# in5omnia/Image_Segmentation

Hardware: AMD Instinct MI355X
Metric: images/sec (fwd+bwd) U-Net 3-class 256x256; IoU parity vs CPU ref (higher is better)
Workload: dtype bf16; 1 GPU; unet(3,3) train step (fwd + ce + bwd + grad all-reduce + AdamW), B=32/GPU 3x256x256, BASELINE config 2; global_batch=32, parallelism=dp1, rccl_ranks=0, rehearsal=False

## Files before the change

image_segmentation_amd/csrc/wgrad.hip:

```cpp
#include <stdlib.h>
#include <type_traits>
#include "common.hpp"
#include "segk_internal.h"
#include "../../include/segk.h"

namespace {

template <int I, int N, typename F> __device__ __forceinline__ void static_for(F&& f) {
  if constexpr (I < N) {
    f(std::integral_constant<int, I>{});
    static_for<I + 1, N>(f);
  }
}

template <typename T, int GEO, int WC = 1> struct WG {
  static constexpr bool BF = (sizeof(T) == 2);
  static constexpr int R = (GEO == 2) ? (BF ? (WC == 4 ? 8 : 4) : 2) : (BF ? 8 : 4);
  static constexpr int NTAPS = GEO == 0 ? 9 : (GEO == 1 ? 1 : 4);
  static constexpr int PH = GEO == 0 ? R + 2 : (GEO == 1 ? R : 2 * R);
  static constexpr int PW = GEO == 0 ? 18 : (GEO == 1 ? 16 : 32);
  static constexpr int BLKP = 32 * (int)sizeof(T);
  static constexpr int PPB = BLKP / 16;
  static constexpr int NDZ = R * 16;
  static constexpr int NPP = PH * PW;
};

__device__ __forceinline__ int tap_pixel(int geo, int tap, int r, int x) {
  if (geo == 0) return (r + tap / 3) * 18 + x + tap % 3;
  if (geo == 1) return r * 16 + x;
  return (2 * r + (tap >> 1)) * 32 + 2 * x + (tap & 1);
}

template <typename T, int GEO, int WC, int WI>
__global__ __launch_bounds__((WC * WI > 4 ? WC * WI : 4) * 64, (sizeof(T) == 2 ? 2 : 1)) void wgrad_kernel(const WgradArgs a) {
  using G = WG<T, GEO, WC>;
  using E = ET<T>;
  constexpr int NT = (WC * WI > 4 ? WC * WI : 4) * 64;
  constexpr int R = G::R, NTAPS = G::NTAPS, BLKP = G::BLKP, PPB = G::PPB;
  constexpr int DZ_PIECES = G::NDZ * WC * PPB, PA_PIECES = G::NPP * WI * PPB;
  constexpr int NDL = (DZ_PIECES + NT - 1) / NT, NPL = (PA_PIECES + NT - 1) / NT;
  constexpr int DZ_BYTES = WC * G::NDZ * BLKP;

  extern __shared__ __attribute__((aligned(16))) char smem[];
  char* const dzs = smem;
  char* const pas = smem + DZ_BYTES;

  const int tid = threadIdx.x, lane = tid & 63, wave = tid >> 6;
  const int H = a.H, W = a.W;
  const int tiles_x = (W + 15) >> 4, tiles_y = (H + R - 1) / R;
  const int ntiles = a.B * tiles_y * tiles_x;

  const int KT = (a.CA + a.CB) / (32 * WI), NCT = (a.CD / (32 * WC)) * KT;
  const int lid = xcd_remap(blockIdx.x, gridDim.x);
  const int s = lid / NCT, ct = lid - s * NCT;
  const int n0 = (ct / KT) * 32 * WC, k0 = (ct % KT) * 32 * WI;

  const T* src; int SC, kc0;
  if (k0 < a.CA) { src = (const T*)a.srcA; SC = a.CA; kc0 = k0; }
  else { src = (const T*)a.srcB; SC = a.CB; kc0 = k0 - a.CA; }
  const bool pro = (a.scale != nullptr);
  const int FH = GEO == 2 ? 2 * H : H, FW = GEO == 2 ? 2 * W : W;

  static_assert(NT % (WC * PPB) == 0 && NT % (WI * PPB) == 0, "channel slot must be thread-invariant");
  const int dcc = tid % (WC * PPB), pcc = tid % (WI * PPB);
  int d_pix[NDL], p_pix[NPL];
#pragma unroll
  for (int i = 0; i < NDL; ++i) {
    const int q = tid + i * NT;
    d_pix[i] = q < DZ_PIECES ? q / (WC * PPB) : -1;
  }
#pragma unroll
  for (int i = 0; i < NPL; ++i) {
    const int q = tid + i * NT;
    p_pix[i] = q < PA_PIECES ? q / (WI * PPB) : -1;
  }
  float psc[E::VEC], psh[E::VEC];
  if (pro) {
#pragma unroll
    for (int j = 0; j < E::VEC; ++j) {
      psc[j] = a.scale[kc0 + pcc * E::VEC + j];
      psh[j] = a.shift[kc0 + pcc * E::VEC + j];
    }
  }

  uint4 dreg[NDL], preg[NPL];
  bool pok[NPL];
  auto prefetch = [&](int t) {
    const int b = t / (tiles_y * tiles_x);
    const int rem = t - b * tiles_y * tiles_x;
    const int y0 = (rem / tiles_x) * R, x0 = (rem % tiles_x) * 16;
#pragma unroll
    for (int i = 0; i < NDL; ++i) {
      uint4 v = make_uint4(0, 0, 0, 0);
      if (d_pix[i] >= 0) {
        const int gy = y0 + (d_pix[i] >> 4), gx = x0 + (d_pix[i] & 15);
        if (gy < H && gx < W)
          v = *(const uint4*)((const T*)a.dz + ((size_t)(b * H + gy) * W + gx) * a.CD + n0 + dcc * E::VEC);
      }
      dreg[i] = v;
    }
#pragma unroll
    for (int i = 0; i < NPL; ++i) {
      pok[i] = false;
      uint4 v = make_uint4(0, 0, 0, 0);
      if (p_pix[i] >= 0) {
        const int py = p_pix[i] / G::PW, px = p_pix[i] - py * G::PW;
        int gy, gx;
        if (GEO == 0) { gy = y0 + py - 1; gx = x0 + px - 1; }
        else if (GEO == 1) { gy = y0 + py; gx = x0 + px; }
        else { gy = 2 * y0 + py; gx = 2 * x0 + px; }
        if (gy >= 0 && gy < FH && gx >= 0 && gx < FW) {
          pok[i] = true;
          v = *(const uint4*)(src + ((size_t)(b * FH + gy) * FW + gx) * SC + kc0 + pcc * E::VEC);
        }
      }
      preg[i] = v;
    }
  };
  auto stage = [&]() {
#pragma unroll
    for (int i = 0; i < NDL; ++i)
      if (d_pix[i] >= 0) {
        const int blk = dcc / PPB, c16 = dcc - blk * PPB;
        *(uint4*)(dzs + blk * (G::NDZ * BLKP) + d_pix[i] * BLKP + c16 * 16) = dreg[i];
      }
#pragma unroll
    for (int i = 0; i < NPL; ++i)
      if (p_pix[i] >= 0) {
        const int blk = pcc / PPB, c16 = pcc - blk * PPB;
        uint4 v = make_uint4(0, 0, 0, 0);
        if (pok[i]) {
          v = preg[i];
          if (pro) {
            float f[E::VEC];
            unpack16<T>(v, f);
#pragma unroll
            for (int j = 0; j < E::VEC; ++j) f[j] = fmaxf(fmaf(f[j], psc[j], psh[j]), 0.f);
            v = pack16<T>(f);
          }
        }
        *(uint4*)(pas + blk * (G::NPP * BLKP) + p_pix[i] * BLKP + c16 * 16) = v;
      }
  };

  const bool computes = wave < WC * WI;
  const int wc = wave / WI, wi = wave - wc * WI;
  f32x16 acc[NTAPS];
#pragma unroll
  for (int t = 0; t < NTAPS; ++t)
#pragma unroll
    for (int r = 0; r < 16; ++r) acc[t][r] = 0.f;

  const char* const dzb = dzs + wc * (G::NDZ * BLKP);
  const char* const pab = pas + wi * (G::NPP * BLKP);

  int t = s;
  if (t < ntiles) prefetch(t);
  for (; t < ntiles; t += a.S) {
    stage();
    __syncthreads();
    if (t + a.S < ntiles) prefetch(t + a.S);
    if (computes) {
      if constexpr (G::BF) {
        const int g = lane >> 4, i16 = lane & 15, q = i16 >> 2, p = i16 & 3;
        const int gsub = g & 1, h = g >> 1;
        const int coff = (16 * gsub + 4 * p) * 2;
        if constexpr (GEO == 2) {
          typedef __attribute__((address_space(3))) s16x4* lds_v4;
          const int xa = 8 * h + q;
          bf16x8 fa[R], fb[2][NTAPS];
          auto rd_b = [&](int r, bf16x8 (&F)[NTAPS]) {
#pragma unroll
            for (int tp = 0; tp < NTAPS; ++tp) {
              const int p0 = tap_pixel(GEO, tp, r, xa), p1 = tap_pixel(GEO, tp, r, xa + 4);
              const s16x4 b0 = __builtin_amdgcn_ds_read_tr16_b64_v4i16((lds_v4)(pab + p0 * BLKP + coff));
              const s16x4 b1 = __builtin_amdgcn_ds_read_tr16_b64_v4i16((lds_v4)(pab + p1 * BLKP + coff));
              F[tp] = __builtin_bit_cast(bf16x8, __builtin_shufflevector(b0, b1, 0, 1, 2, 3, 4, 5, 6, 7));
            }
          };
#pragma unroll
          for (int r = 0; r < R; ++r) {
            const s16x4 a0 = __builtin_amdgcn_ds_read_tr16_b64_v4i16((lds_v4)(dzb + (r * 16 + xa) * BLKP + coff));
            const s16x4 a1 = __builtin_amdgcn_ds_read_tr16_b64_v4i16((lds_v4)(dzb + (r * 16 + xa + 4) * BLKP + coff));
            fa[r] = __builtin_bit_cast(bf16x8, __builtin_shufflevector(a0, a1, 0, 1, 2, 3, 4, 5, 6, 7));
          }
          rd_b(0, fb[0]);
#pragma unroll
          for (int r = 0; r < R; ++r) {
            if (r + 1 < R) rd_b(r + 1, fb[(r + 1) & 1]);
            __builtin_amdgcn_sched_barrier(0);
#pragma unroll
            for (int tp = 0; tp < NTAPS; ++tp) acc[tp] = __builtin_amdgcn_mfma_f32_32x32x16_bf16(fa[r], fb[r & 1][tp], acc[tp], 0, 0, 0);
            __builtin_amdgcn_sched_barrier(0);
          }
        } else {
      #pragma unroll
        for (int r = 0; r < R; ++r) {
          const int xa = 8 * h + q;
          typedef __attribute__((address_space(3))) s16x4* lds_v4;
          const s16x4 a0 = __builtin_amdgcn_ds_read_tr16_b64_v4i16((lds_v4)(dzb + (r * 16 + xa) * BLKP + coff));
          const s16x4 a1 = __builtin_amdgcn_ds_read_tr16_b64_v4i16((lds_v4)(dzb + (r * 16 + xa + 4) * BLKP + coff));
          const bf16x8 fa = __builtin_bit_cast(bf16x8, __builtin_shufflevector(a0, a1, 0, 1, 2, 3, 4, 5, 6, 7));
#pragma unroll
          for (int tp = 0; tp < NTAPS; ++tp) {
            const int p0 = tap_pixel(GEO, tp, r, xa), p1 = tap_pixel(GEO, tp, r, xa + 4);
            const s16x4 b0 = __builtin_amdgcn_ds_read_tr16_b64_v4i16((lds_v4)(pab + p0 * BLKP + coff));
            const s16x4 b1 = __builtin_amdgcn_ds_read_tr16_b64_v4i16((lds_v4)(pab + p1 * BLKP + coff));
            const bf16x8 fb = __builtin_bit_cast(bf16x8, __builtin_shufflevector(b0, b1, 0, 1, 2, 3, 4, 5, 6, 7));
            acc[tp] = __builtin_amdgcn_mfma_f32_32x32x16_bf16(fa, fb, acc[tp], 0, 0, 0);
          }
        }
        }
      } else {
        const int i32 = lane & 31, h = lane >> 5;
#pragma unroll
        for (int r = 0; r < R; ++r) {
#pragma unroll
          for (int kp = 0; kp < 8; ++kp) {
            const int x = 2 * kp + h;
            const float fa = *(const float*)(dzb + (r * 16 + x) * BLKP + i32 * 4);
#pragma unroll
            for (int tp = 0; tp < NTAPS; ++tp) {
              const float fb = *(const float*)(pab + tap_pixel(GEO, tp, r, x) * BLKP + i32 * 4);
              acc[tp] = __builtin_amdgcn_mfma_f32_32x32x2f32(fa, fb, acc[tp], 0, 0, 0);
            }
          }
        }
      }
    }
    __syncthreads();
  }

  if (computes) {
    const int K = a.CA + a.CB;
    const int col = lane & 31, lh = lane >> 5;
    float* const slab = a.slabs + (size_t)s * a.CD * NTAPS * K;
#pragma unroll
    for (int tp = 0; tp < NTAPS; ++tp)
#pragma unroll
      for (int r = 0; r < 16; ++r) {
        const int row = (r & 3) + 8 * (r >> 2) + 4 * lh;
        slab[((size_t)(n0 + wc * 32 + row) * NTAPS + tp) * K + k0 + wi * 32 + col] = acc[tp][r];
      }
  }
}

#ifdef SEGK_WGRAD_STAMPS
__device__ unsigned long long g_wstamps[256 * 8 * 8];
#endif
template <int WC, int WI, bool PRO, bool RAG>
__global__ __launch_bounds__((WC * WI > 4 ? WC * WI : 4) * 64, 2) void wgrad_dma_kernel(const WgradArgs a) {
  typedef bf16_t T;
  constexpr int NWV = WC * WI > 4 ? WC * WI : 4;
  constexpr int R = 8, NTAPS = 9, BLKP = 64;
  constexpr int WU = PRO ? WI : WC, WV = PRO ? WC : WI;
  constexpr int NU = R * 16, NV = 192;
  constexpr int UB = WU * NU * BLKP, VB = WV * NV * BLKP, BUF = UB + VB;
  constexpr int NINSTR = WU * 8 + WV * 12;
  extern __shared__ __attribute__((aligned(16))) char smem[];

  const int tid = threadIdx.x, lane = tid & 63;
  const int wave = __builtin_amdgcn_readfirstlane(tid >> 6);
  const int H = a.H, W = a.W;
  const int tiles_x = (W + 15) >> 4, tiles_y = (H + R - 1) / R;
  const int ntiles = a.B * tiles_y * tiles_x;
  const int KT = (a.CA + a.CB) / (32 * WI), NCT = (a.CD / (32 * WC)) * KT;
  const int lid = xcd_remap(blockIdx.x, gridDim.x);
  const int s = lid / NCT, ct = lid - s * NCT;
  const int n0 = (ct / KT) * 32 * WC, k0 = (ct % KT) * 32 * WI;

  const T* srck; int SCk, kc0;
  if (k0 < a.CA) { srck = (const T*)a.srcA; SCk = a.CA; kc0 = k0; }
  else { srck = (const T*)a.srcB; SCk = a.CB; kc0 = k0 - a.CA; }
  const T* const ubase = PRO ? srck + kc0 : (const T*)a.dz + n0;
  const int UC = PRO ? SCk : a.CD;
  const T* const vbase = PRO ? (const T*)a.dz + n0 : srck + kc0;
  const int VC = PRO ? a.CD : SCk;
  const char* const zeros = (const char*)a.zeros;

  const int lp = lane >> 2, lc = lane & 3;
  constexpr int NI = (NINSTR + NWV - 1) / NWV;
  int poff[NI];
  int pyx[RAG ? NI : 1];
  unsigned pflag[(NI + 5) / 6];
#pragma unroll
  for (int q = 0; q < (NI + 5) / 6; ++q) pflag[q] = 0u;
#pragma unroll
  for (int i = 0; i < NI; ++i) {
    const int j = min(wave + NWV * i, NINSTR - 1);
    if (j < WU * 8) {
      const int blk = j >> 3, r = j & 7;
      poff[i] = ((r * W + lp) * UC + blk * 32 + lc * 8) * 2;
      if constexpr (RAG) pyx[i] = ((r + 1) << 8) | (lp + 1);
    } else {
      const int jj = j - WU * 8;
      const int blk = jj / 12, ch = jj - blk * 12;
      const int pp = ch * 16 + lp;
      const int py = pp / 18, px = pp - py * 18;
      poff[i] = (((py - 1) * W + (px - 1)) * VC + blk * 32 + lc * 8) * 2;
      const unsigned f = (py == 0 ? 1u : 0u) | (py == 9 ? 2u : 0u) | (px == 0 ? 4u : 0u) | (px == 17 ? 8u : 0u) |
                         (pp >= 180 ? 16u : 0u);
      pflag[i / 6] |= f << (5 * (i % 6));
      if constexpr (RAG) pyx[i] = (py << 8) | px;
    }
  }
  auto issue_tile = [&](int t, int bufsel) {
    const int bimg = t / (tiles_y * tiles_x);
    const int rem = t - bimg * tiles_y * tiles_x;
    const int y0 = (rem / tiles_x) * R, x0 = (rem % tiles_x) * 16;
    {
      const unsigned out = (y0 == 0 ? 1u : 0u) | (y0 + R >= H ? 2u : 0u) | (x0 == 0 ? 4u : 0u) | (x0 + 16 >= W ? 8u : 0u) | 16u;
      const size_t pix0 = (size_t)(bimg * H + y0) * W + x0;
      const char* const ub0 = (const char*)(ubase + pix0 * UC);
      const char* const vb0 = (const char*)(vbase + pix0 * VC);
      char* const bb = smem + bufsel * BUF;
      const char* const zsrc = zeros + lc * 16;
#pragma unroll
      for (int i = 0; i < NI; ++i) {
        const int j = wave + NWV * i;
        if (j >= NINSTR) break;
        const bool is_u = j < WU * 8;
        const int jj = j - WU * 8;
        char* const dst = is_u ? bb + (j >> 3) * (NU * BLKP) + (j & 7) * 1024
                               : bb + UB + (jj / 12) * (NV * BLKP) + (jj % 12) * 1024;
        const char* const base = is_u ? ub0 : vb0;
        bool bad;
        if constexpr (RAG) {
          const int py = pyx[i] >> 8, px = pyx[i] & 255;
          bad = (((pflag[i / 6] >> (5 * (i % 6))) & 16u) != 0u) | (py == 0 ? y0 == 0 : py > H - y0) |
                (px == 0 ? x0 == 0 : px > W - x0);
        } else {
          bad = ((pflag[i / 6] >> (5 * (i % 6))) & out) != 0u;
        }
        const char* const src = bad ? zsrc : base + (ptrdiff_t)poff[i];
        __builtin_amdgcn_global_load_lds((const __attribute__((address_space(1))) void*)src,
                                         (__attribute__((address_space(3))) void*)dst, 16, 0, 0);
      }
    }
  };

  const bool computes = wave < WC * WI;
  const int wc = wave / WI, wi = wave - wc * WI;
  const int wu = PRO ? wi : wc, wv = PRO ? wc : wi;
  f32x16 acc[NTAPS];
#pragma unroll
  for (int t = 0; t < NTAPS; ++t)
#pragma unroll
    for (int r = 0; r < 16; ++r) acc[t][r] = 0.f;

  const int g = lane >> 4, i16 = lane & 15, q = i16 >> 2, p = i16 & 3;
  const int gsub = g & 1, h = g >> 1;
  const int coff = (16 * gsub + 4 * p) * 2;
  const int xa = 8 * h + q;
  float psc = 1.f, psh = 0.f;
  if (PRO) {
    const int c = kc0 + wu * 32 + 16 * gsub + i16;
    psc = a.scale[c];
    psh = a.shift[c];
  }
  typedef __attribute__((ext_vector_type(8))) short s16x8;
  auto frag_rd = [&](s16x8& dst, int vaddr, auto OFFc) {
    constexpr int OFF = decltype(OFFc)::value;
    s16x4 f0, f1;
    asm volatile("ds_read_b64_tr_b16 %0, %1 offset:%2" : "=v"(f0) : "v"(vaddr), "n"(OFF));
    asm volatile("ds_read_b64_tr_b16 %0, %1 offset:%2" : "=v"(f1) : "v"(vaddr), "n"(OFF + 4 * BLKP));
    dst = __builtin_shufflevector(f0, f1, 0, 1, 2, 3, 4, 5, 6, 7);
  };
  typedef short s16x2 __attribute__((ext_vector_type(2)));
  auto transform = [&](s16x8 v, unsigned vmask) {
    const uint4 raw = __builtin_bit_cast(uint4, v);
    float f[8];
    unpack16<T>(raw, f);
    unsigned o[4];
#pragma unroll
    for (int i = 0; i < 4; ++i) {
      const float x0 = fmaf(f[2 * i], psc, psh), x1 = fmaf(f[2 * i + 1], psc, psh);
      unsigned pk;
      pk = cvt_pk_bf16(x0, x1);
      o[i] = __builtin_bit_cast(unsigned, __builtin_elementwise_max(__builtin_bit_cast(s16x2, pk), (s16x2){0, 0}));
    }
    if (vmask != 0xffu) {
#pragma unroll
      for (int i = 0; i < 4; ++i)
        o[i] &= ((vmask >> (2 * i)) & 1 ? 0x0000ffffu : 0u) | ((vmask >> (2 * i + 1)) & 1 ? 0xffff0000u : 0u);
    }
    return __builtin_bit_cast(s16x8, make_uint4(o[0], o[1], o[2], o[3]));
  };

#ifdef SEGK_WGRAD_STAMPS
  unsigned long long wst[3] = {0, 0, 0}, wlast, wt0;
  asm volatile("s_waitcnt lgkmcnt(0)\n\ts_memtime %0\n\ts_waitcnt lgkmcnt(0)" : "=s"(wlast)::"memory");
  wt0 = wlast;
#define WSTAMP(i) do { unsigned long long t_; asm volatile("s_memtime %0\n\ts_waitcnt lgkmcnt(0)" : "=s"(t_)::"memory"); \
                       wst[i] += t_ - wlast; wlast = t_; } while (0)
#else
#define WSTAMP(i) do {} while (0)
#endif
  int t = s, cur = 0;
  if (t < ntiles) issue_tile(t, 0);
  asm volatile("s_waitcnt vmcnt(0)" ::: "memory");
  __syncthreads();
  WSTAMP(2);
#ifndef WGRAD_STAGGER_ROW
#define WGRAD_STAGGER_ROW 1
#endif
  constexpr int SROW = (NWV == 8) ? WGRAD_STAGGER_ROW : -1;
  const bool late_issue = SROW >= 0 && wave >= NWV / 2;
  for (; t < ntiles; t += a.S) {
    const bool has_next = t + a.S < ntiles;
    if (has_next && !late_issue) issue_tile(t + a.S, cur ^ 1);
    if (computes) {
      unsigned xmask = 0xffu, rows_ok = R;
      if (PRO) {
        const int bimg = t / (tiles_y * tiles_x);
        const int rem = t - bimg * tiles_y * tiles_x;
        const int y0 = (rem / tiles_x) * R, x0 = (rem % tiles_x) * 16;
        rows_ok = (unsigned)min(R, H - y0);
        xmask = 0;
#pragma unroll
        for (int j = 0; j < 8; ++j)
          xmask |= (x0 + 8 * h + j < W ? 1u : 0u) << j;
      }
      const int ua = cur * BUF + wu * (NU * BLKP) + xa * BLKP + coff;
      const int va = cur * BUF + UB + wv * (NV * BLKP) + xa * BLKP + coff;
      s16x8 fv[3][3], fu[2];
      frag_rd(fu[0], ua, std::integral_constant<int, 0>{});
      static_for<0, 9>([&](auto IC) {
        constexpr int y = decltype(IC)::value / 3, kx = decltype(IC)::value % 3;
        frag_rd(fv[y][kx], va, std::integral_constant<int, (y * 18 + kx) * BLKP>{});
      });
      if (PRO) {
        asm volatile("s_waitcnt lgkmcnt(15)" ::: "memory");
        __builtin_amdgcn_sched_barrier(0);
        fu[0] = transform(fu[0], rows_ok > 0 ? xmask : 0u);
      }
      static_for<0, R>([&](auto RC) {
        constexpr int r = decltype(RC)::value;
        if constexpr (r + 1 < R) frag_rd(fu[(r + 1) & 1], ua, std::integral_constant<int, (r + 1) * 16 * BLKP>{});
        asm volatile("s_waitcnt lgkmcnt(%0)" ::"n"((r == 0 ? 12 : 6) + (r + 1 < R ? 2 : 0)) : "memory");
        __builtin_amdgcn_sched_barrier(0);
        const bf16x8 fur = __builtin_bit_cast(bf16x8, fu[r & 1]);
#pragma unroll
        for (int kx = 0; kx < 3; ++kx) {
          const bf16x8 fvr = __builtin_bit_cast(bf16x8, fv[r % 3][kx]);
          const int ti = PRO ? 8 - kx : kx;
          acc[ti] = PRO ? __builtin_amdgcn_mfma_f32_32x32x16_bf16(fvr, fur, acc[ti], 0, 0, 0)
                        : __builtin_amdgcn_mfma_f32_32x32x16_bf16(fur, fvr, acc[ti], 0, 0, 0);
        }
        __builtin_amdgcn_sched_barrier(0);
        if constexpr (r + 1 < R) {
          static_for<0, 3>([&](auto KC) {
            constexpr int kx = decltype(KC)::value;
            frag_rd(fv[r % 3][kx], va, std::integral_constant<int, ((r + 3) * 18 + kx) * BLKP>{});
          });
        }
        asm volatile("s_waitcnt lgkmcnt(%0)" ::"n"(r + 1 < R ? 8 : 0) : "memory");
        __builtin_amdgcn_sched_barrier(0);
#pragma unroll
        for (int ky = 1; ky < 3; ++ky)
#pragma unroll
          for (int kx = 0; kx < 3; ++kx) {
            const bf16x8 fvr = __builtin_bit_cast(bf16x8, fv[(r + ky) % 3][kx]);
            const int ti = PRO ? 8 - (ky * 3 + kx) : ky * 3 + kx;
            acc[ti] = PRO ? __builtin_amdgcn_mfma_f32_32x32x16_bf16(fvr, fur, acc[ti], 0, 0, 0)
                          : __builtin_amdgcn_mfma_f32_32x32x16_bf16(fur, fvr, acc[ti], 0, 0, 0);
          }
        __builtin_amdgcn_sched_barrier(0);
        if constexpr (r == SROW) {
          if (has_next && late_issue) issue_tile(t + a.S, cur ^ 1);
          __builtin_amdgcn_sched_barrier(0);
        }
        if constexpr (PRO && r + 1 < R) {
          asm volatile("s_waitcnt lgkmcnt(6)" ::: "memory");
          __builtin_amdgcn_sched_barrier(0);
          fu[(r + 1) & 1] = transform(fu[(r + 1) & 1], (unsigned)(r + 1) < rows_ok ? xmask : 0u);
        }
      });
    }
    WSTAMP(0);
    asm volatile("s_waitcnt vmcnt(0)" ::: "memory");
    WSTAMP(1);
    __syncthreads();
    WSTAMP(2);
    cur ^= 1;
  }

  if (computes) {
    const int K = a.CA + a.CB;
    const int col = lane & 31, lh = lane >> 5;
    float* const slab = a.slabs + (size_t)s * a.CD * NTAPS * K;
#pragma unroll
    for (int tp = 0; tp < NTAPS; ++tp)
#pragma unroll
      for (int r = 0; r < 16; ++r) {
        const int row = (r & 3) + 8 * (r >> 2) + 4 * lh;
        slab[((size_t)(n0 + wc * 32 + row) * NTAPS + tp) * K + k0 + wi * 32 + col] = acc[tp][r];
      }
  }
#ifdef SEGK_WGRAD_STAMPS
  {
    unsigned long long t_;
    asm volatile("s_waitcnt vmcnt(0)\n\ts_memtime %0\n\ts_waitcnt lgkmcnt(0)" : "=s"(t_)::"memory");
    if (lane == 0 && blockIdx.x < 256) {
      unsigned long long* o = g_wstamps + ((size_t)blockIdx.x * 8 + wave) * 8;
      o[0] = wst[0]; o[1] = wst[1]; o[2] = wst[2]; o[3] = t_ - wlast; o[4] = t_ - wt0;
    }
  }
#endif
}

template <int WC, int WI, bool PRO, bool RAG>
int launch_dma(const WgradArgs& a, hipStream_t st) {
  constexpr int WU = PRO ? WI : WC, WV = PRO ? WC : WI;
  constexpr size_t lds = 2 * ((size_t)WU * 128 * 64 + (size_t)WV * 192 * 64);
  static_assert(lds <= 160 * 1024, "wgrad_dma: LDS exceeds 160 KiB");
  const int NCT = (a.CD / (32 * WC)) * ((a.CA + a.CB) / (32 * WI));
  auto kern = wgrad_dma_kernel<WC, WI, PRO, RAG>;
  static bool attr_set[SEGK_MAX_DEVICES] = {};
  const int dev_ = segk_device_index();
  if (!attr_set[dev_]) {
    if (hipFuncSetAttribute((const void*)kern, hipFuncAttributeMaxDynamicSharedMemorySize, 160 * 1024) != hipSuccess)
      SEGK_FAIL(-3, "wgrad_dma: cannot raise dynamic LDS limit");
    attr_set[dev_] = true;
  }
  hipLaunchKernelGGL(kern, dim3(a.S * NCT), dim3((WC * WI > 4 ? WC * WI : 4) * 64), lds, st, a);
#ifdef SEGK_WGRAD_STAMPS
  { void* sp = nullptr; if (hipGetSymbolAddress(&sp, HIP_SYMBOL(g_wstamps)) == hipSuccess) (void)hipMemcpyAsync(a.slabs, sp, sizeof(unsigned long long) * 256 * 8 * 8, hipMemcpyDeviceToDevice, st); }
#endif
  SEGK_CHECK_LAUNCH("wgrad_dma");
  return 0;
}

template <int WC, int WI>
int launch_dma_pro(const WgradArgs& a, hipStream_t st) {
  const bool rag = a.H % 8 != 0 || a.W % 16 != 0;
  if (rag) return a.scale ? launch_dma<WC, WI, true, true>(a, st) : launch_dma<WC, WI, false, true>(a, st);
  return a.scale ? launch_dma<WC, WI, true, false>(a, st) : launch_dma<WC, WI, false, false>(a, st);
}

template <typename T, int GEO, int WC, int WI>
int launch_cfg(const WgradArgs& a, hipStream_t st) {
  using G = WG<T, GEO, WC>;
  const size_t lds = (size_t)WC * G::NDZ * G::BLKP + (size_t)WI * G::NPP * G::BLKP;
  const int NCT = (a.CD / (32 * WC)) * ((a.CA + a.CB) / (32 * WI));
  auto kern = wgrad_kernel<T, GEO, WC, WI>;
  static bool attr_set[SEGK_MAX_DEVICES] = {};
  const int dev_ = segk_device_index();
  if (!attr_set[dev_]) {
    if (hipFuncSetAttribute((const void*)kern, hipFuncAttributeMaxDynamicSharedMemorySize, 160 * 1024) != hipSuccess)
      SEGK_FAIL(-3, "wgrad: cannot raise dynamic LDS limit");
    attr_set[dev_] = true;
  }
  hipLaunchKernelGGL(kern, dim3(a.S * NCT), dim3((WC * WI > 4 ? WC * WI : 4) * 64), lds, st, a);
#ifdef SEGK_WGRAD_STAMPS
  { void* sp = nullptr; if (hipGetSymbolAddress(&sp, HIP_SYMBOL(g_wstamps)) == hipSuccess) (void)hipMemcpyAsync(a.slabs, sp, sizeof(unsigned long long) * 256 * 8 * 8, hipMemcpyDeviceToDevice, st); }
#endif
  SEGK_CHECK_LAUNCH("wgrad");
  return 0;
}

template <typename T, int GEO>
int launch_geo(const WgradArgs& a, hipStream_t st) {
  const bool wc2 = a.CD % 64 == 0;
  const bool wi2 = a.CA % 64 == 0 && a.CB % 64 == 0;
  if constexpr (GEO == 0 && sizeof(T) == 2) {
    if (a.zeros) {
      if (segk_wgrad_wc(a.CD, a.CA, a.CB, 0, SEGK_DT_BF16) == 4) return launch_dma_pro<4, 2>(a, st);
      if (wc2 && wi2) return launch_dma_pro<2, 2>(a, st);
      if (wc2) return launch_dma_pro<2, 1>(a, st);
      if (wi2) return launch_dma_pro<1, 2>(a, st);
      return launch_dma_pro<1, 1>(a, st);
    }
  }
  if constexpr (GEO == 2 && sizeof(T) == 2) {
    if (segk_wgrad_wc(a.CD, a.CA, a.CB, 2, SEGK_DT_BF16) == 4) return launch_cfg<T, GEO, 4, 2>(a, st);
  }
  if (wc2 && wi2) return launch_cfg<T, GEO, 2, 2>(a, st);
  if (wc2) return launch_cfg<T, GEO, 2, 1>(a, st);
  if (wi2) return launch_cfg<T, GEO, 1, 2>(a, st);
  return launch_cfg<T, GEO, 1, 1>(a, st);
}

template <typename T>
int launch_t(const WgradArgs& a, int geo, hipStream_t st) {
  if (geo == 0) return launch_geo<T, 0>(a, st);
  if (geo == 1) return launch_geo<T, 1>(a, st);
  return launch_geo<T, 2>(a, st);
}

}

int segk_wgrad_wc(int CD, int CA, int CB, int geo, int dtype) {
  static const bool off = getenv("SEGK_WGRAD_NO_WC4") != nullptr;
  if ((geo == 0 || geo == 2) && dtype == SEGK_DT_BF16 && !off && CD % 128 == 0 && CA % 64 == 0 && CB % 64 == 0) return 4;
  return CD % 64 == 0 ? 2 : 1;
}
int segk_wgrad_split(int tiles, int CD, int CA, int CB, int geo, int dtype) {
  if (tiles <= 0 || CD <= 0 || CA <= 0 || CB < 0 || CD % 32 || CA % 32 || CB % 32) return 0;
  const int wc = segk_wgrad_wc(CD, CA, CB, geo, dtype);
  const int wi = (CA % 64 == 0 && CB % 64 == 0) ? 2 : 1;
  const int nct = (CD / (32 * wc)) * ((CA + CB) / (32 * wi));
  const int target = wc == 4 ? 256 : 512;
  if (wc == 4 && geo == 2) tiles = (tiles + 1) / 2;
  int S = nct < target ? target / nct : 1;
  if (S > tiles) S = tiles;
  return S < 1 ? 1 : S;
}

int segk_wgrad_tiles(int B, int H, int W, int geo, int dtype) {
  const bool bf = dtype == SEGK_DT_BF16;
  const int R = geo == 2 ? (bf ? 4 : 2) : (bf ? 8 : 4);
  if (B <= 0 || H <= 0 || W <= 0) return 0;
  const long long n = (long long)B * cdiv(H, R) * cdiv(W, 16);
  return n > 0x7fffffffLL ? 0 : (int)n;
}

int segk_wgrad_launch(const WgradArgs& a, int geo, int dtype, hipStream_t st) {
  SEGK_REQUIRE(dtype == SEGK_DT_F32 || dtype == SEGK_DT_BF16, "wgrad: bad dtype %d", dtype);
  SEGK_REQUIRE(geo >= 0 && geo <= 2, "wgrad: bad geometry %d", geo);
  SEGK_REQUIRE(a.dz && a.srcA && a.slabs, "wgrad: null pointer");
  SEGK_REQUIRE(a.B > 0 && a.H > 0 && a.W > 0, "wgrad: bad shape");
  SEGK_REQUIRE(a.CD > 0 && a.CD % 32 == 0 && a.CA > 0 && a.CA % 32 == 0 && a.CB >= 0 && a.CB % 32 == 0,
               "wgrad: channel counts must be multiples of 32 (CD=%d CA=%d CB=%d)", a.CD, a.CA, a.CB);
  SEGK_REQUIRE((a.CB == 0) == (a.srcB == nullptr), "wgrad: second source mismatch");
  SEGK_REQUIRE(!(a.scale && a.CB) && ((a.scale == nullptr) == (a.shift == nullptr)), "wgrad: bad BN prologue");
  SEGK_REQUIRE(a.S >= 1 && a.S <= 65535, "wgrad: bad split-K factor %d", a.S);
  SEGK_REQUIRE((long long)a.B * a.H * a.W * 4 < 2147483647LL, "wgrad: pixel index overflows int32");
  return dtype == SEGK_DT_BF16 ? launch_t<bf16_t>(a, geo, st) : launch_t<float>(a, geo, st);
}
```

Baseline: 2815 images/sec.

## Add 16x16x32 MFMA wgrad kernel with transposed LDS reads for 3x3 convs

Adds a new weight-gradient kernel for bf16 3x3 convolutions on the 4x2 wave configuration. It uses 16x16x32 bf16 MFMA with ds_read_b64_tr_b16 transposed LDS fragment reads, DMA global-to-LDS double buffering and a hand-scheduled software pipeline that interleaves LDS reads with MFMA groups. The kernel is selected by default when scale is off and the tile dims divide evenly, and SEGK_WGRAD_OLD restores the old path. Debug timestamps also gain a real-time counter. Register pressure from 36 f32x4 accumulators and the rigid lgkmcnt scheduling are the risks.

```diff
diff --git a/image_segmentation_amd/csrc/wgrad.hip b/image_segmentation_amd/csrc/wgrad.hip
--- a/image_segmentation_amd/csrc/wgrad.hip
+++ b/image_segmentation_amd/csrc/wgrad.hip
@@ -388,8 +388,8 @@
   };
 
 #ifdef SEGK_WGRAD_STAMPS
-  unsigned long long wst[3] = {0, 0, 0}, wlast, wt0;
-  asm volatile("s_waitcnt lgkmcnt(0)\n\ts_memtime %0\n\ts_waitcnt lgkmcnt(0)" : "=s"(wlast)::"memory");
+  unsigned long long wst[3] = {0, 0, 0}, wlast, wt0, wr0;
+  asm volatile("s_waitcnt lgkmcnt(0)\n\ts_memtime %0\n\ts_memrealtime %1\n\ts_waitcnt lgkmcnt(0)" : "=s"(wlast), "=s"(wr0)::"memory");
   wt0 = wlast;
 #define WSTAMP(i) do { unsigned long long t_; asm volatile("s_memtime %0\n\ts_waitcnt lgkmcnt(0)" : "=s"(t_)::"memory"); \
                        wst[i] += t_ - wlast; wlast = t_; } while (0)
@@ -499,11 +499,237 @@
   }
 #ifdef SEGK_WGRAD_STAMPS
   {
-    unsigned long long t_;
-    asm volatile("s_waitcnt vmcnt(0)\n\ts_memtime %0\n\ts_waitcnt lgkmcnt(0)" : "=s"(t_)::"memory");
+    unsigned long long t_, r_;
+    asm volatile("s_waitcnt vmcnt(0)\n\ts_memtime %0\n\ts_memrealtime %1\n\ts_waitcnt lgkmcnt(0)" : "=s"(t_), "=s"(r_)::"memory");
     if (lane == 0 && blockIdx.x < 256) {
       unsigned long long* o = g_wstamps + ((size_t)blockIdx.x * 8 + wave) * 8;
-      o[0] = wst[0]; o[1] = wst[1]; o[2] = wst[2]; o[3] = t_ - wlast; o[4] = t_ - wt0;
+      o[0] = wst[0]; o[1] = wst[1]; o[2] = wst[2]; o[3] = t_ - wlast; o[4] = t_ - wt0; o[5] = r_ - wr0;
+    }
+  }
+#endif
+}
+
+__global__ __launch_bounds__(512, 2) void wgrad_mf16_kernel(const WgradArgs a) {
+  typedef bf16_t T;
+  constexpr int WC = 4, WI = 2, NWV = 8;
+  constexpr int R = 8, NTAPS = 9, BLKP = 64;
+  constexpr int NU = R * 16, NV = 192;
+  constexpr int UB = WC * NU * BLKP, VB = WI * NV * BLKP, BUF = UB + VB;
+  constexpr int NINSTR = WC * 8 + WI * 12;
+  constexpr int NI = NINSTR / NWV;
+  static_assert(NINSTR % NWV == 0, "every wave issues the same number of DMA pieces");
+  constexpr int TOG = 65536;
+  static_assert(BUF <= TOG, "tile buffer exceeds 64 KiB");
+  extern __shared__ __attribute__((aligned(16))) char smem[];
+
+  const int tid = threadIdx.x, lane = tid & 63;
+  const int wave = __builtin_amdgcn_readfirstlane(tid >> 6);
+  const int H = a.H, W = a.W;
+  const int tiles_x = W >> 4, tiles_y = H >> 3;
+  const int ntiles = a.B * tiles_y * tiles_x;
+  const int KT = (a.CA + a.CB) / (32 * WI), NCT = (a.CD / (32 * WC)) * KT;
+  const int lid = xcd_remap(blockIdx.x, gridDim.x);
+  const int s = lid / NCT, ct = lid - s * NCT;
+  const int n0 = (ct / KT) * 32 * WC, k0 = (ct % KT) * 32 * WI;
+
+  const T* srck; int SCk, kc0;
+  if (k0 < a.CA) { srck = (const T*)a.srcA; SCk = a.CA; kc0 = k0; }
+  else { srck = (const T*)a.srcB; SCk = a.CB; kc0 = k0 - a.CA; }
+  const T* const ubase = (const T*)a.dz + n0;
+  const int UC = a.CD;
+  const T* const vbase = srck + kc0;
+  const int VC = SCk;
+  const char* const zeros = (const char*)a.zeros;
+
+  static_assert(NWV == 8 && WC * 8 == 32 && NI == 7, "piece map of the 4 x 2 workgroup");
+  constexpr int NIV = NI - 4;
+  const int lp = lane >> 2, lc = lane & 3;
+  const int uoff = ((wave * W + lp) * UC + (lc ^ (((lp >> 3) & 1) << 1)) * 8) * 2;
+  int voff[NIV];
+#pragma unroll
+  for (int i = 0; i < NIV; ++i) {
+    const int jj = wave + NWV * i;
+    const int blk = jj / 12, ch = jj - blk * 12;
+    const int pp = ch * 16 + lp;
+    const int py = pp / 18, px = pp - py * 18;
+    const int f = (py == 0 ? 1 : 0) | (py >= 9 ? 2 : 0) | (px == 0 ? 4 : 0) | (px == 17 ? 8 : 0);
+    voff[i] = ((((py - 1) * W + (px - 1)) * VC + blk * 32 + (lc ^ (((px >> 3) & 1) << 1)) * 8) * 2) | f;
+  }
+  auto issue_tile = [&](int t, int bufsel) {
+    const int bimg = t / (tiles_y * tiles_x);
+    const int rem = t - bimg * tiles_y * tiles_x;
+    const int y0 = (rem / tiles_x) * R, x0 = (rem % tiles_x) * 16;
+    const int out = (y0 == 0 ? 1 : 0) | (y0 + R >= H ? 2 : 0) | (x0 == 0 ? 4 : 0) | (x0 + 16 >= W ? 8 : 0);
+    const size_t pix0 = (size_t)(bimg * H + y0) * W + x0;
+    const char* const ub0 = (const char*)(ubase + pix0 * UC);
+    const char* const vb0 = (const char*)(vbase + pix0 * VC);
+    char* const bb = smem + bufsel * TOG;
+#pragma unroll
+    for (int i = 0; i < 4; ++i)
+      __builtin_amdgcn_global_load_lds((const __attribute__((address_space(1))) void*)(ub0 + 64 * i + uoff),
+                                       (__attribute__((address_space(3))) void*)(bb + i * (NU * BLKP) + wave * 1024), 16, 0, 0);
+#pragma unroll
+    for (int i = 0; i < NIV; ++i) {
+      const int jj = wave + NWV * i;
+      char* const dst = bb + UB + (jj / 12) * (NV * BLKP) + (jj % 12) * 1024;
+      int vo = voff[i];
+      asm volatile("" : "+v"(vo));
+      const char* const src = (vo & out) != 0 ? zeros + lc * 16 : vb0 + (ptrdiff_t)(vo & ~15);
+      __builtin_amdgcn_global_load_lds((const __attribute__((address_space(1))) void*)src,
+                                       (__attribute__((address_space(3))) void*)dst, 16, 0, 0);
+    }
+  };
+
+  const int wc = wave / WI, wi = wave - wc * WI;
+  f32x4 acc[NTAPS][2][2];
+#pragma unroll
+  for (int tp = 0; tp < NTAPS; ++tp)
+#pragma unroll
+    for (int c = 0; c < 2; ++c)
+#pragma unroll
+      for (int d = 0; d < 2; ++d) acc[tp][c][d] = (f32x4){0.f, 0.f, 0.f, 0.f};
+
+  const int g = lane >> 4, i16 = lane & 15, q = i16 >> 2, p = i16 & 3;
+  const int rr = g >> 1, hc = g & 1;
+  const int ul = wc * (NU * BLKP) + (16 * rr + 8 * hc + q) * BLKP + 8 * p;
+  const int vl = UB + wi * (NV * BLKP) + (18 * rr + 8 * hc + q) * BLKP + 8 * p;
+  int ua[2] = {ul + 32 * hc, ul + 32 * (hc ^ 1)};
+  int va[3][2];
+#pragma unroll
+  for (int kx = 0; kx < 3; ++kx)
+#pragma unroll
+    for (int x = 0; x < 2; ++x) va[kx][x] = vl + 32 * (x ^ hc ^ (q + kx >= 4 ? 1 : 0));
+
+  typedef __attribute__((ext_vector_type(8))) short s16x8;
+  auto frag_rd = [&](s16x8& dst, int vaddr0, int vaddr1, auto OFFc) {
+    constexpr int OFF = decltype(OFFc)::value;
+    s16x4 f0, f1;
+    asm volatile("ds_read_b64_tr_b16 %0, %1 offset:%2" : "=v"(f0) : "v"(vaddr0), "n"(OFF));
+    asm volatile("ds_read_b64_tr_b16 %0, %1 offset:%2" : "=v"(f1) : "v"(vaddr1), "n"(OFF + 4 * BLKP));
+    dst = __builtin_shufflevector(f0, f1, 0, 1, 2, 3, 4, 5, 6, 7);
+  };
+  s16x8 fu[2][2];
+  s16x8 fv[2][3][2];
+  auto read_u = [&](auto SC) {
+    constexpr int st = decltype(SC)::value;
+    frag_rd(fu[st & 1][0], ua[0], ua[0], std::integral_constant<int, st * 32 * BLKP>{});
+    frag_rd(fu[st & 1][1], ua[1], ua[1], std::integral_constant<int, st * 32 * BLKP>{});
+  };
+  auto read_v = [&](auto MC) {
+    constexpr int m = decltype(MC)::value;
+    static_for<0, 6>([&](auto IC) {
+      constexpr int kx = decltype(IC)::value >> 1, d = decltype(IC)::value & 1;
+      frag_rd(fv[m % 2][kx][d], va[0][d], va[kx][d], std::integral_constant<int, (m * 18 + kx) * BLKP>{});
+    });
+  };
+  auto flip = [&]() {
+#pragma unroll
+    for (int x = 0; x < 2; ++x) {
+      ua[x] ^= TOG;
+#pragma unroll
+      for (int kx = 0; kx < 3; ++kx) va[kx][x] ^= TOG;
+    }
+  };
+  auto mfma_ky = [&](auto KYC, auto SC) {
+    constexpr int ky = decltype(KYC)::value, st = decltype(SC)::value;
+#pragma unroll
+    for (int kx = 0; kx < 3; ++kx)
+#pragma unroll
+      for (int c = 0; c < 2; ++c)
+#pragma unroll
+        for (int d = 0; d < 2; ++d)
+          acc[ky * 3 + kx][c][d] = __builtin_amdgcn_mfma_f32_16x16x32_bf16(__builtin_bit_cast(bf16x8, fu[st & 1][c]),
+                                                                          __builtin_bit_cast(bf16x8, fv[(2 * st + ky) % 2][kx][d]),
+                                                                          acc[ky * 3 + kx][c][d], 0, 0, 0);
+    __builtin_amdgcn_sched_barrier(0);
+  };
+  using I0 = std::integral_constant<int, 0>;
+  using I1 = std::integral_constant<int, 1>;
+  using I2 = std::integral_constant<int, 2>;
+  using I3 = std::integral_constant<int, 3>;
+
+#ifdef SEGK_WGRAD_STAMPS
+  unsigned long long wst[3] = {0, 0, 0}, wlast, wt0, wr0;
+  asm volatile("s_waitcnt lgkmcnt(0)\n\ts_memtime %0\n\ts_memrealtime %1\n\ts_waitcnt lgkmcnt(0)" : "=s"(wlast), "=s"(wr0)::"memory");
+  wt0 = wlast;
+#endif
+  auto boundary = [&]() {
+    WSTAMP(0);
+    asm volatile("s_waitcnt vmcnt(0)" ::: "memory");
+    WSTAMP(1);
+    __builtin_amdgcn_sched_barrier(0);
+    __builtin_amdgcn_s_barrier();
+    __builtin_amdgcn_sched_barrier(0);
+    WSTAMP(2);
+  };
+
+  int t = s, cur = 0;
+  if (t < ntiles) issue_tile(t, 0);
+  asm volatile("s_waitcnt vmcnt(0)" ::: "memory");
+  __syncthreads();
+  WSTAMP(2);
+  read_u(I0{});
+  read_v(I0{});
+  read_v(I1{});
+  const bool late_issue = wave >= NWV / 2;
+  for (; t < ntiles; t += a.S) {
+    const bool has_next = t + a.S < ntiles;
+    if (has_next && !late_issue) issue_tile(t + a.S, cur ^ 1);
+    static_for<0, 4>([&](auto SC) {
+      constexpr int st = decltype(SC)::value;
+      asm volatile("s_waitcnt lgkmcnt(12)" ::: "memory");
+      __builtin_amdgcn_sched_barrier(0);
+      mfma_ky(I0{}, SC);
+      asm volatile("s_waitcnt lgkmcnt(0)" ::: "memory");
+      __builtin_amdgcn_sched_barrier(0);
+      read_v(std::integral_constant<int, 2 * st + 2>{});
+      if constexpr (st < 3) read_u(std::integral_constant<int, st + 1>{});
+      __builtin_amdgcn_sched_barrier(0);
+      mfma_ky(I1{}, SC);
+      asm volatile("s_waitcnt lgkmcnt(%0)" ::"n"(st < 3 ? 4 : 0) : "memory");
+      __builtin_amdgcn_sched_barrier(0);
+      if constexpr (st < 3) read_v(std::integral_constant<int, 2 * st + 3>{});
+      __builtin_amdgcn_sched_barrier(0);
+      mfma_ky(I2{}, SC);
+      if constexpr (st == 0) {
+        if (has_next && late_issue) issue_tile(t + a.S, cur ^ 1);
+        __builtin_amdgcn_sched_barrier(0);
+      }
+      if constexpr (st == 3) {
+        boundary();
+        flip();
+        read_u(I0{});
+        read_v(I0{});
+        read_v(I1{});
+        __builtin_amdgcn_sched_barrier(0);
+      }
+    });
+    cur ^= 1;
+  }
+  asm volatile("s_waitcnt lgkmcnt(0)" ::: "memory");
+
+  {
+    const int K = a.CA + a.CB;
+    float* const slab = a.slabs + (size_t)s * a.CD * NTAPS * K;
+#pragma unroll
+    for (int tp = 0; tp < NTAPS; ++tp)
+#pragma unroll
+      for (int c = 0; c < 2; ++c)
+#pragma unroll
+        for (int d = 0; d < 2; ++d)
+#pragma unroll
+          for (int i = 0; i < 4; ++i) {
+            const int co = n0 + wc * 32 + 16 * c + 4 * g + i, ci = k0 + wi * 32 + 16 * d + i16;
+            slab[((size_t)co * NTAPS + tp) * K + ci] = acc[tp][c][d][i];
+          }
+  }
+#ifdef SEGK_WGRAD_STAMPS
+  {
+    unsigned long long t_, r_;
+    asm volatile("s_waitcnt vmcnt(0)\n\ts_memtime %0\n\ts_memrealtime %1\n\ts_waitcnt lgkmcnt(0)" : "=s"(t_), "=s"(r_)::"memory");
+    if (lane == 0 && blockIdx.x < 256) {
+      unsigned long long* o = g_wstamps + ((size_t)blockIdx.x * 8 + wave) * 8;
+      o[0] = wst[0]; o[1] = wst[1]; o[2] = wst[2]; o[3] = t_ - wlast; o[4] = t_ - wt0; o[5] = r_ - wr0;
     }
   }
 #endif
@@ -538,6 +764,25 @@
   return a.scale ? launch_dma<WC, WI, true, false>(a, st) : launch_dma<WC, WI, false, false>(a, st);
 }
 
+int launch_mf16(const WgradArgs& a, hipStream_t st) {
+  constexpr size_t lds = 65536 + ((size_t)4 * 128 * 64 + (size_t)2 * 192 * 64);
+  static_assert(lds <= 160 * 1024, "wgrad_mf16: LDS exceeds 160 KiB");
+  const int NCT = (a.CD / 128) * ((a.CA + a.CB) / 64);
+  static bool attr_set[SEGK_MAX_DEVICES] = {};
+  const int dev_ = segk_device_index();
+  if (!attr_set[dev_]) {
+    if (hipFuncSetAttribute((const void*)wgrad_mf16_kernel, hipFuncAttributeMaxDynamicSharedMemorySize, 160 * 1024) != hipSuccess)
+      SEGK_FAIL(-3, "wgrad_mf16: cannot raise dynamic LDS limit");
+    attr_set[dev_] = true;
+  }
+  hipLaunchKernelGGL(wgrad_mf16_kernel, dim3(a.S * NCT), dim3(512), lds, st, a);
+#ifdef SEGK_WGRAD_STAMPS
+  { void* sp = nullptr; if (hipGetSymbolAddress(&sp, HIP_SYMBOL(g_wstamps)) == hipSuccess) (void)hipMemcpyAsync(a.slabs, sp, sizeof(unsigned long long) * 256 * 8 * 8, hipMemcpyDeviceToDevice, st); }
+#endif
+  SEGK_CHECK_LAUNCH("wgrad_mf16");
+  return 0;
+}
+
 template <typename T, int GEO, int WC, int WI>
 int launch_cfg(const WgradArgs& a, hipStream_t st) {
   using G = WG<T, GEO, WC>;
@@ -565,7 +810,11 @@
   const bool wi2 = a.CA % 64 == 0 && a.CB % 64 == 0;
   if constexpr (GEO == 0 && sizeof(T) == 2) {
     if (a.zeros) {
-      if (segk_wgrad_wc(a.CD, a.CA, a.CB, 0, SEGK_DT_BF16) == 4) return launch_dma_pro<4, 2>(a, st);
+      if (segk_wgrad_wc(a.CD, a.CA, a.CB, 0, SEGK_DT_BF16) == 4) {
+        static const bool old = getenv("SEGK_WGRAD_OLD") != nullptr;
+        if (!old && !a.scale && a.H % 8 == 0 && a.W % 16 == 0) return launch_mf16(a, st);
+        return launch_dma_pro<4, 2>(a, st);
+      }
       if (wc2 && wi2) return launch_dma_pro<2, 2>(a, st);
       if (wc2) return launch_dma_pro<2, 1>(a, st);
       if (wi2) return launch_dma_pro<1, 2>(a, st);
```

New measurement: 2839 images/sec (median of 6 runs). About the same (+0.8%).
